# jbrea/BayesianOptimization.jl

Hardware: AMD Instinct MI355X
Metric: acquisition-candidates/sec (N=3000,d=8) (higher is better)
Workload: dtype f64

## Files before the change

bayesianoptimization.jl_amd/csrc/bohip.hip:

```cpp
#include "../../include/bohip.h"
#include "../../include/bohip_paths.h"
#include "../../include/bohip_fit.h"
#include "kernels_linalg.hip"
#include "kernels_chol.hip"
#include "kernels_exec.hip"
#include "kernels_score.hip"
#include "kernels_batch.hip"
#include "kernels_sample.hip"
#include "kernels_path.hip"
#include "kernels_ascent.hip"
#include "kernels_fit.hip"
#include "kernels_small.hip"
#include "direct_l.h"

#include <algorithm>
#include <atomic>
#include <chrono>
#include <cerrno>
#include <cmath>
#include <cstdio>
#include <cstring>
#include <limits>
#include <mutex>
#include <fcntl.h>
// ... 63 lines not shown
    int* dpieces = nullptr;
    std::vector<int> hpieces;
    int n_pieces = 0, pieces_T = -1;
    int64_t pieces_cap = 0;
    int64_t pieces_alpha = -1;
    int64_t kst_rows = 0;
    int64_t chunk_now = 0;
    int64_t score_launches = 0;
    double *dVT = nullptr, *dUT = nullptr;
    int64_t vt_rows = 0;
    double *dq = nullptr, *dmu_raw = nullptr, *dXs = nullptr, *dmu = nullptr, *dvar = nullptr, *dscore = nullptr;
    int64_t q_cap = 0, r_cap = 0, xs_cap = 0;
    Best *dblock_best = nullptr, *dbest = nullptr;
    int64_t bb_cap = 0;
    unsigned* dfz_cnt = nullptr;
    Best* dfz_best = nullptr;
    int64_t fz_cap = 0;
    bool fz_dirty = false;
    char* dpr = nullptr;
    size_t pr_bytes = 0;
    std::vector<int> hpr_pieces;
    int* pr_pieces_at = nullptr;
    unsigned* hprune_stat = nullptr;
    int prune_skip = 0;
    double* dBV = nullptr;
    int64_t bv_rows = 0, bv_ld = 0;
    char* dbatch = nullptr;
    size_t batch_bytes = 0;
    double* dgrad = nullptr;
    double asc_ftol_abs = 0.0, asc_xtol_rel = 0.0, asc_stopval = INFINITY;
    double asc_maxtime = 0.0;
    int64_t batch_hint = 0;
    double* dsplit = nullptr;
    int64_t split_cap = 0;
    const SmallFold* asc_fold = nullptr;
    bool asc_fold_done = false;
    const unsigned* asc_go = nullptr;
    double* dgparts = nullptr;
    unsigned* dgcount = nullptr;
    double* dsm = nullptr;
    size_t sm_bytes = 0;
    unsigned* dsm_cnt = nullptr;
    int sm_cnt_T = 0;
    double* hpin = nullptr;
    double* dschur = nullptr;
    AscentState asc{};
// ... 1844 lines not shown
    hipLaunchKernelGGL(k_split_combine_v, dim3((unsigned)R), dim3(256), 0, g->stream, g->dsplit, Rc * ld, ld, sp.kz, N, g->dq,
                       g->dmu_raw, want_u ? g->dVT : nullptr, ld);
    HIPCHK(hipGetLastError());
    t_end(g);
    g->q_tiles = 0;
    if (want_u) {
        t_begin(g, "split_U");
        GemmNTParams u{};
        u.A = g->dVT; u.lda = ld; u.B = g->dWT; u.ldb = ld; u.C = g->dsplit; u.ldc = ld;
        u.zA = (int64_t)sp.kz * KC; u.zB = (int64_t)sp.kz * KC; u.zC = Rc * ld;
        u.mt = (int)(Rc / TILE); u.nt64 = 2 * T; u.kc = sp.kz; u.alpha = 1.0; u.beta = 0.0;
        u.klo_from_n = 1; u.kz = sp.kz; u.ktot = T * (TILE / KC);
        CHK(launch_gemm_nt(g, u, sp.nsl));
        hipLaunchKernelGGL(k_split_combine_u, dim3((unsigned)R), dim3(256), 0, g->stream, g->dsplit, Rc * ld, ld, sp.kz, sp.nsl, N,
                           g->dUT, ld);
        HIPCHK(hipGetLastError());
        t_end(g);
    }
    return 0;
}

constexpr int PRUNE_K1 = 64;
constexpr int PRUNE_ROWS_CAP = 256;
constexpr int64_t PRUNE_R_MAX = 8192;
static int prune_tiles(int T) {
    if (g_prune_m >= 0) return g_prune_m < T ? g_prune_m : 0;
    int m = 2;
    while ((double)m * (m + 1) < 0.02 * T * (T + 1)) ++m;
    return m < T ? m : 0;
}
static std::vector<int> rows_halves(const std::vector<int>& pieces) {
    std::vector<int> out;
    if (!g_ks8) return out;
    for (int c : pieces) {
        const int rt = c & 0xffff, mode = c >> 16;
        if (mode == PIECE_UPPER_SOLO) out.push_back(rt | 1 << 17);
        else if (mode == PIECE_WHOLE) { out.push_back(rt | 1 << 16); out.push_back(rt); }
        else return {};
    }
    std::stable_sort(out.begin(), out.end(), [](int a, int b) {
        return 8 * (a & 0xffff) + ((a >> 16) & 1) * 4 > 8 * (b & 0xffff) + ((b >> 16) & 1) * 4;
    });
    return out;
}
static int rows_halves_from(const std::vector<int>& hv, int t0) {
    int n = 0;
    while (n < (int)hv.size() && (hv[n] & 0xffff) >= t0) ++n;
    return n;
}
static int launch_trigemm_rows(bohip_gp* g, const double* KsT, const int* halves, int NH, const int* list, const unsigned* cnt,
                               int cnt_max, double* q, int64_t ldq, double* mu) {
    if (NH <= 0 || cnt_max <= 0) return 0;
    RowsParams rp{};
    rp.W = g->dW; rp.ldw = g->ld; rp.KsT = KsT; rp.ldk = g->ld; rp.list = list; rp.cnt = cnt; rp.cnt_max = cnt_max;
    rp.halves = halves; rp.NH = NH; rp.G = (cnt_max + RS_COLS - 1) / RS_COLS; rp.alpha_row = g->n; rp.q = q; rp.ldq = ldq; rp.mu = mu;
    hipLaunchKernelGGL(k_trigemm_rows, dim3((unsigned)(8 * ((NH + 7) / 8) * rp.G)), dim3(RS_THREADS), RS_LDS_BYTES, g->stream, rp);
    HIPCHK(hipGetLastError());
    return 0;
}
static int launch_trigemm_on(bohip_gp* g, const double* KsT, const int* pieces, int NP, int CT, double* q, int64_t ldq, double* mu_raw,
                             FuseParams fz) {
    const int n_local = (CT + 7) / 8;
    if (NP <= 0 || CT <= 0) return 0;
    if (g->timing && g->dclk) fz.clk = g->dclk;
    if (g_ks8)
        hipLaunchKernelGGL(k_trigemm_sq<2>, dim3(8 * n_local * NP), dim3(GEMM_THREADS_8), glds3_lds_bytes<4>(), g->stream, g->dW,
                           g->ld, KsT, g->ld, pieces, NP, CT, g->n, q, ldq, mu_raw, (int64_t)0, nullptr, g->ld, fz);
    else
        hipLaunchKernelGGL(k_trigemm_sq<1>, dim3(8 * n_local * NP), dim3(GEMM_THREADS), glds3_lds_bytes<4>(), g->stream, g->dW,
                           g->ld, KsT, g->ld, pieces, NP, CT, g->n, q, ldq, mu_raw, (int64_t)0, nullptr, g->ld, fz);
    HIPCHK(hipGetLastError());
    return 0;
}
static int pruned_pass(bohip_gp* g, const double* dXs, int64_t R, int m, const AcqParams& ap, Best* d_best, int64_t best_off,
                       double* ub_host = nullptr) {
    CHK(one_time_kernel_setup());
    if (!g->hprune_stat) {
        HIPCHK(hipHostMalloc((void**)&g->hprune_stat, 64, hipHostMallocDefault));
        g->hprune_stat[0] = 0u;
    }
    const int64_t N = g->n, Npad = round_up(N + 1, TILE), Rpad = round_up(R, TILE) + TILE, ld = g->ld;
    const int T = (int)(Npad / TILE);
    const int64_t P = Npad / 64;
    CHK(ensure_pieces(g, T, N));
    std::vector<int> pa, pb;
    for (int c : g->hpieces) ((c & 0xffff) < m ? pa : pb).push_back(c);
    auto al = [](size_t b) { return (b + 255) / 256 * 256; };
    const size_t o_ks = 0, o_q2 = o_ks + al((size_t)Rpad * ld * 8), o_mu2 = o_q2 + al((size_t)2 * T * Rpad * 8),
                 o_ub = o_mu2 + al((size_t)Rpad * 8), o_l1 = o_ub + al((size_t)Rpad * 8), o_l2 = o_l1 + al((size_t)PRUNE_K1 * 4),
                 o_mark = o_l2 + al((size_t)Rpad * 4), o_cnt = o_mark + al((size_t)Rpad * 4), o_rec = o_cnt + 256,
                 o_parts = o_rec + 256, o_pc = o_parts + al((size_t)2 * P * Rpad * 8), total = o_pc + al((3 * g->hpieces.size() + 8) * 4);
    bool fresh = false;
    if (g->pr_bytes < total) {
        fresh = true;
        if (g->dpr) { HIPCHK(hipStreamSynchronize(g->stream)); HIPCHK(hipFree(g->dpr)); g->dpr = nullptr; g->pr_bytes = 0; }
        HIPCHK(hipMalloc(&g->dpr, total));
        g->pr_bytes = total;
    }
// ... 27 lines not shown
    t_end(g);
    t_begin(g, "trigemm_sq");
    FuseParams fz{};
    fz.T = T;
    CHK(launch_trigemm_on(g, g->dKsT, pcs, (int)pa.size(), (int)((R + CTILE - 1) / CTILE), g->dq, Rpad, g->dmu_raw, fz));
    PruneBound bd{};
    bd.parts = kp.parts; bd.P = P; bd.ldp = Rpad; bd.Npad = Npad; bd.q = g->dq; bd.ldq = Rpad; bd.R = R; bd.m = m;
    bd.sigma2 = sigma2; bd.beta = g->beta; bd.ap = ap; bd.ub = ub;
    hipLaunchKernelGGL(k_prune_bound, dim3((unsigned)((R + 63) / 64)), dim3(64), 0, g->stream, bd);
    if (ub_host) {
        t_end(g);
        HIPCHK(hipGetLastError());
        HIPCHK(hipMemcpyAsync(ub_host, ub, (size_t)R * 8, hipMemcpyDeviceToHost, g->stream));
        HIPCHK(hipStreamSynchronize(g->stream));
        return 0;
    }
    static_assert(PRUNE_R_MAX <= (int64_t)SELECT_THREADS * SELECT_PER, "k_prune_select holds the whole batch in one workgroup");
    hipLaunchKernelGGL(k_prune_select, dim3(1), dim3(SELECT_THREADS), 0, g->stream, (const double*)ub, R, k1, l1, mark, cnt, rec);
    HIPCHK(hipGetLastError());
    PruneFinish pf{};
    pf.q = g->dq; pf.ldq = Rpad; pf.q2 = q2; pf.ldq2 = Rpad; pf.mu2 = mu2; pf.m = m; pf.T = T; pf.sigma2 = sigma2; pf.beta = g->beta;
    pf.ap = ap; pf.rec = rec;
    const int* hvd = pcs + pa.size() + pb.size();
    for (int round = 0; round < 2; ++round) {
        const int* list = round == 0 ? l1 : l2;
        const unsigned* c = cnt + round;
        const int64_t cap = round == 0 ? k1 : R - k1;
        if (cap > 0 && nh > 0 && cap <= PRUNE_ROWS_CAP) {
            CHK(launch_trigemm_rows(g, g->dKsT, hvd, nh, list, c, (int)cap, q2, Rpad, mu2));
        } else if (cap > 0) {
            const int sq_min = nh > 0 ? PRUNE_ROWS_CAP : -1;
            hipLaunchKernelGGL(k_prune_gather, dim3((unsigned)cap), dim3(256), 0, g->stream, list, c, (const double*)g->dKsT, ld, Npad, ks2,
                               sq_min, cnt + 2);
            fz.live = cnt + 2;
            CHK(launch_trigemm_on(g, ks2, pcs + pa.size(), (int)pb.size(), (int)((cap + CTILE - 1) / CTILE), q2, Rpad, mu2, fz));
            if (nh > 0) CHK(launch_trigemm_rows(g, g->dKsT, hvd, nh, list, c, PRUNE_ROWS_CAP, q2, Rpad, mu2));
        }
        pf.list = list; pf.cnt = c;
        pf.best_out = round == 1 ? d_best : nullptr; pf.best_off = (long long)best_off;
        pf.stat = round == 1 ? g->hprune_stat : nullptr;
        pf.ub = ub; pf.mark = mark; pf.R = R; pf.list2 = round == 0 ? l2 : nullptr; pf.cnt2 = cnt + 1;
        hipLaunchKernelGGL(k_prune_finish, dim3(1), dim3(256), 0, g->stream, pf);
        HIPCHK(hipGetLastError());
    }
    t_end(g);
    return 0;
}

constexpr int PRUNE_BACKOFF = 31;
static bool prune_wanted(bohip_gp* g, int64_t R) {
    if (g->prune_skip > 0) { --g->prune_skip; return false; }
    if (g->hprune_stat) {
        const unsigned n2 = __atomic_load_n(g->hprune_stat, __ATOMIC_RELAXED);
        if ((int64_t)n2 > R / 8) {
            __atomic_store_n(g->hprune_stat, 0u, __ATOMIC_RELAXED);
            g->prune_skip = PRUNE_BACKOFF - 1;
            return false;
        }
    }
    return true;
}

static int score_core(bohip_gp* g, int acq_id, const double* acq_params, const double* dXs, int64_t R, double* d_mu,
                      double* d_var, double* d_score, Best* d_best, int64_t best_off = 0) {
    if (g->n == 0) return fail(BOHIP_E_STATE, "model has no observations");
    CHK(ensure_fresh(g));
    CHK(ensure_score_scratch(g, R));
    AcqParams ap{acq_id, 0.0, 0.0};
    if (acq_params) {
        if (acq_id != BOHIP_ACQ_MAXMEAN) ap.p0 = acq_params[0];
        if (acq_id == BOHIP_ACQ_MI) ap.p1 = acq_params[1];
    } else if (acq_id != BOHIP_ACQ_MAXMEAN) {
        return fail(BOHIP_E_ARG, "acq_params required for this acquisition");
    }
    if (path_R(g, R) <= small_limit(g) && R <= SMALL_MAX) {
        CHK(one_time_kernel_setup());
        return small_posterior(g, dXs, 0, R, false, ap, d_mu, d_var, d_score, d_best, best_off);
    }
    const SplitPlan sp = split_plan(g, R);
    if (sp.nsl > 0) {
        CHK(split_posterior(g, dXs, R, sp, false));
    } else if (int m = prune_tiles((int)(round_up(g->n + 1, TILE) / TILE));
               m > 0 && g_fuse_finish && d_best && !d_mu && !d_var && !d_score && R <= PRUNE_R_MAX && R <= g->chunk_now &&
               g->batch_hint == 0 && prune_wanted(g, R)) {
        return pruned_pass(g, dXs, R, m, ap, d_best, best_off);
    } else if (g_fuse_finish) {
        FuseParams fz{};
        fz.tile_cnt = g->dfz_cnt; fz.total_cnt = g->dfz_cnt + g->fz_cap; fz.tile_best = g->dfz_best;
        fz.tiles_total = (int)((R + CTILE - 1) / CTILE); fz.R_total = R;
        fz.sigma2 = std::exp(2.0 * g->logsig); fz.beta = g->beta; fz.ap = ap;
        fz.mu_out = d_mu; fz.var_out = d_var; fz.score_out = d_score; fz.best_out = d_best; fz.best_off = best_off;
        if (g->fz_dirty) HIPCHK(hipMemsetAsync(g->dfz_cnt, 0, (size_t)(g->fz_cap + 1 + 16) * sizeof(unsigned), g->stream));
        g->fz_dirty = true;
        const int rc = posterior_pass(g, dXs, R, fz);
        if (rc == 0) g->fz_dirty = false;
        return rc;
    } else {
        CHK(posterior_pass(g, dXs, R));
    }
    const int64_t Npad = round_up(g->n + 1, TILE), Rpad = round_up(R, TILE) + TILE;
    const int T = (int)(Npad / TILE);
    const int nb = (int)((R + 255) / 256);
    t_begin(g, "score");
    hipLaunchKernelGGL(k_score, dim3(nb), dim3(256), 0, g->stream, g->dq, Rpad, g->q_tiles, g->dmu_raw, R,
                       std::exp(2.0 * g->logsig), g->beta, ap, d_mu, d_var, d_score, d_best ? g->dblock_best : nullptr);
    if (d_best) hipLaunchKernelGGL(k_argmax_final, dim3(1), dim3(256), 0, g->stream, g->dblock_best, nb, d_best, (long long)best_off);
    HIPCHK(hipGetLastError());
    t_end(g);
// ... 1696 lines not shown
    one_time_kernel_setup();
    std::vector<int> ps;
    trigemm_pieces(T, alpha_row, ps);
    for (int i = 0; i < (int)ps.size() && i < cap; ++i) out[i] = ps[i];
    return (int)ps.size();
}
int bohip_debug_prune_bounds(bohip_gp* g, int acq_id, const double* acq_params, const double* Xs, int64_t R, double* ub) {
    if (!g || R <= 0 || !Xs || !ub || acq_id < 0 || acq_id > BOHIP_ACQ_MAXMEAN) return fail(BOHIP_E_ARG, "bad arguments");
    HIPCHK(hipSetDevice(g->device));
    if (g->n == 0) return fail(BOHIP_E_STATE, "model has no observations");
    CHK(ensure_fresh(g));
    CHK(ensure_xs(g, R));
    CHK(ensure_score_scratch(g, R));
    AcqParams ap{acq_id, 0.0, 0.0};
    if (acq_params && acq_id != BOHIP_ACQ_MAXMEAN) ap.p0 = acq_params[0];
    if (acq_params && acq_id == BOHIP_ACQ_MI) ap.p1 = acq_params[1];
    const int m = prune_tiles((int)(round_up(g->n + 1, TILE) / TILE));
    if (m == 0 || R > PRUNE_R_MAX || R > g->chunk_now || (path_R(g, R) <= small_limit(g) && R <= SMALL_MAX) || split_plan(g, R).nsl > 0)
        return fail(BOHIP_E_UNSUPPORTED, "no pruning at this size");
    HIPCHK(hipMemcpyAsync(g->dXs, Xs, (size_t)R * g->d * 8, hipMemcpyHostToDevice, g->stream));
    return pruned_pass(g, g->dXs, R, m, ap, nullptr, 0, ub);
}
int bohip_debug_trigemm_partials(bohip_gp* g, const double* Xs, int64_t R, int path, double* q_out, double* mu_out) {
    if (!g || R <= 0 || !Xs || !q_out || !mu_out || (path != 0 && path != 1)) return fail(BOHIP_E_ARG, "bad arguments");
    HIPCHK(hipSetDevice(g->device));
    if (g->n == 0) return fail(BOHIP_E_STATE, "model has no observations");
    CHK(ensure_fresh(g));
    CHK(ensure_xs(g, R));
    CHK(ensure_score_scratch(g, R));
    if (R > g->chunk_now) return fail(BOHIP_E_UNSUPPORTED, "more than one K*' chunk");
    CHK(one_time_kernel_setup());
    const int64_t N = g->n, Npad = round_up(N + 1, TILE), Rpad = round_up(R, TILE);
    const int T = (int)(Npad / TILE);
    CHK(ensure_pieces(g, T, N));
    const std::vector<int> hv = rows_halves(g->hpieces);
    if (path == 1 && hv.empty()) return fail(BOHIP_E_UNSUPPORTED, "row pieces k_trigemm_rows does not reproduce");
    HIPCHK(hipMemcpyAsync(g->dXs, Xs, (size_t)R * g->d * 8, hipMemcpyHostToDevice, g->stream));
    CHK(launch_kstar_any(g, g->dXs, 0, R, Npad, make_hyper(g)));
    std::vector<double> q((size_t)2 * T * Rpad), mu((size_t)Rpad);
    if (path == 0) {
        CHK(launch_trigemm_on(g, g->dKsT, g->dpieces, g->n_pieces, (int)((R + CTILE - 1) / CTILE), g->dq, Rpad, g->dmu_raw, FuseParams{}));
        HIPCHK(hipMemcpyAsync(q.data(), g->dq, q.size() * 8, hipMemcpyDeviceToHost, g->stream));
        HIPCHK(hipMemcpyAsync(mu.data(), g->dmu_raw, mu.size() * 8, hipMemcpyDeviceToHost, g->stream));
        HIPCHK(hipStreamSynchronize(g->stream));
        for (int t = 0; t < 2 * T; ++t) std::memcpy(q_out + (size_t)t * R, q.data() + (size_t)t * Rpad, (size_t)R * 8);
        std::memcpy(mu_out, mu.data(), (size_t)R * 8);
        return 0;
    }
    std::vector<int> list((size_t)R);
    for (int64_t i = 0; i < R; ++i) list[i] = (int)(R - 1 - i);
    const unsigned n = (unsigned)R;
    char* d = nullptr;
    const size_t o_q = 0, o_mu = o_q + q.size() * 8, o_l = o_mu + mu.size() * 8, o_h = o_l + list.size() * 4, o_c = o_h + hv.size() * 4;
    HIPCHK(hipMalloc(&d, o_c + 16));
    int rc = 0;
    hipMemcpyAsync(d + o_l, list.data(), list.size() * 4, hipMemcpyHostToDevice, g->stream);
    hipMemcpyAsync(d + o_h, hv.data(), hv.size() * 4, hipMemcpyHostToDevice, g->stream);
    hipMemcpyAsync(d + o_c, &n, 4, hipMemcpyHostToDevice, g->stream);
    rc = launch_trigemm_rows(g, g->dKsT, (const int*)(d + o_h), (int)hv.size(), (const int*)(d + o_l), (const unsigned*)(d + o_c), (int)R,
                             (double*)(d + o_q), Rpad, (double*)(d + o_mu));
    hipMemcpyAsync(q.data(), d + o_q, q.size() * 8, hipMemcpyDeviceToHost, g->stream);
    hipMemcpyAsync(mu.data(), d + o_mu, mu.size() * 8, hipMemcpyDeviceToHost, g->stream);
    const hipError_t e = hipStreamSynchronize(g->stream);
    hipFree(d);
    if (rc != 0) return rc;
    if (e != hipSuccess) return fail(BOHIP_E_HIP, hipGetErrorString(e));
    for (int t = 0; t < 2 * T; ++t)
        for (int64_t i = 0; i < R; ++i) q_out[(size_t)t * R + list[i]] = q[(size_t)t * Rpad + i];
    for (int64_t i = 0; i < R; ++i) mu_out[list[i]] = mu[i];
    return 0;
}
int64_t bohip_debug_prune_stat(bohip_gp* g) {
    if (!g || !g->hprune_stat) return -1;
    return (int64_t)__atomic_load_n(g->hprune_stat, __ATOMIC_RELAXED);
}
int bohip_debug_set_chol_inv_g(int g_new) {
    return g_chol_inv_g.exchange(std::min(64, std::max(0, g_new)));
}
int bohip_debug_exec_throughput(bohip_gp* g, unsigned qmask, int hot, int wgs, double* ms_out, double* gflop_out) {
    if (!g || !ms_out || g->n == 0) return BOHIP_E_ARG;
    hipSetDevice(g->device);
    CHK(one_time_kernel_setup());
    const int T = (int)(round_up(g->n + 1, TILE) / TILE);
    if (T <= 3) return BOHIP_E_UNSUPPORTED;
    std::vector<ExTask> all, run;
    int qb[EX_NQ + 1], qb2[EX_NQ + 1];
    exec_task_list(g->dL, g->dS, g->dW, g->dWT, g->dchol_flags, g->ld, T, g_chol_nsf, g_chol_inv_g, all, qb);
    double fl = 0.0;
    qb2[0] = 0;
    for (int qi = 0; qi < EX_NQ; ++qi) {
        if ((qmask >> qi) & 1u)
            for (int i = qb[qi]; i < qb[qi + 1]; ++i) {
                ExTask t = all[i];
                for (int d = 0; d < EX_NDEP; ++d) { t.dep_idx[d] = EX_NONE; t.dep_want[d] = 0; }
                t.sig_idx[0] = t.sig_idx[1] = EX_NONE;
                t.kc_split = 0; t.dep2_idx[0] = t.dep2_idx[1] = EX_NONE;
                if (hot && (qi == EX_QBULK || qi == EX_QWAVE)) { t.A = g->dS; t.B = g->dS + (int64_t)TILE * g->ld; }
// ... 61 lines not shown
```

bayesianoptimization.jl_amd/csrc/kernels_score.hip:

```cpp
#include "gemm_core.h"

namespace bohip {

template <bool LOW>
__device__ __forceinline__ double cov_from_r_fast(int fam, double sigma2, double r) {
    if constexpr (LOW) {
        return matern_lo_k(fam, sigma2, r);
    } else {
        if (fam == FAM_M52) {
            const double R = sqrt(r), s = sqrt(5.0) * R;
            return sigma2 * (1.0 + s + 5.0 / 3.0 * r) * exp(-s);
        }
        return sigma2 * exp(-0.5 * r);
    }
}

struct KstarParts {
    const double* alpha;
    double* parts;
    int64_t ldp;
};
__device__ __forceinline__ void swap32(double a, double b, double& x, double& y) {
    const unsigned long long ua = (unsigned long long)__double_as_longlong(a), ub = (unsigned long long)__double_as_longlong(b);
    const auto lo = __builtin_amdgcn_permlane32_swap((unsigned)ua, (unsigned)ub, false, false);
// ... 532 lines not shown
            ub = (mu_up - ap.p0 >= 0.0 ? 1.0 : acq_eval(ap, mu_up, s2)) + 0x1p-38;
            break;
        case ACQ_UCB:
        case ACQ_MI: {
            const double sb = ap.p0 >= 0.0 ? s2 : 0.0;
            const double f = acq_eval(ap, mu_up, sb);
            const double roots = ap.acq == ACQ_UCB ? sqrt(sb) : sqrt(sb + fabs(ap.p1)) + sqrt(fabs(ap.p1));
            ub = f + 0x1p-38 * (fabs(mu_up) + fabs(ap.p0) * roots + 0x1p-1000);
            break;
        }
        default:
            ub = mu_up;
    }
    pb.ub[r] = ub;
}

__device__ __forceinline__ double prune_key(double v) { return v != v ? INFINITY : v; }
__device__ __forceinline__ unsigned long long prune_key_bits(double v) {
    const double k = prune_key(v);
    const unsigned long long b = k == 0.0 ? 0ull : (unsigned long long)__double_as_longlong(k);
    return (b >> 63) ? ~b : b | 0x8000000000000000ull;
}
constexpr int SELECT_THREADS = 1024, SELECT_PER = 8;
__global__ __launch_bounds__(SELECT_THREADS) void k_prune_select(const double* __restrict__ ub, int64_t R, int k1, int* __restrict__ list1,
                                                                 int* __restrict__ mark, unsigned* __restrict__ cnt, Best* __restrict__ rec) {
    __shared__ uint4 hist[3][64];
    __shared__ unsigned long long red[2 * SELECT_THREADS / 64];
    __shared__ unsigned tot[SELECT_THREADS / 64];
    const int t = threadIdx.x, lane = t & 63, wave = t >> 6;
    const int per = (int)((R + SELECT_THREADS - 1) / SELECT_THREADS);
    unsigned long long key[SELECT_PER];
    unsigned long long kmax = 0ull, kmin = ~0ull;
#pragma unroll
    for (int i = 0; i < SELECT_PER; ++i) {
        const int64_t r = (int64_t)t * per + i;
        key[i] = (i < per && r < R) ? prune_key_bits(ub[r]) : 0ull;
        if (key[i]) { kmax = max(kmax, key[i]); kmin = min(kmin, key[i]); }
    }
    for (int o = 32; o > 0; o >>= 1) {
        kmax = max(kmax, __shfl_xor(kmax, o));
        kmin = min(kmin, __shfl_xor(kmin, o));
    }
    if (lane == 0) { red[2 * wave] = kmax; red[2 * wave + 1] = kmin; }
    if (t < 128) (&hist[0][0])[t] = make_uint4(0u, 0u, 0u, 0u);
    __syncthreads();
    for (int w = 0; w < SELECT_THREADS / 64; ++w) { kmax = max(kmax, red[2 * w]); kmin = min(kmin, red[2 * w + 1]); }
// ... 38 lines not shown
    const unsigned mine = (unsigned)ngt | (unsigned)neq << 16;
    unsigned incl = mine;
    for (int o = 1; o < 64; o <<= 1) {
        const unsigned u = __shfl_up(incl, o);
        if (lane >= o) incl += u;
    }
    if (lane == 63) tot[wave] = incl;
    __syncthreads();
    for (int w = 0; w < wave; ++w) incl += tot[w];
    int g = (int)((incl - mine) & 0xffffu), e = (int)((incl - mine) >> 16);
#pragma unroll
    for (int i = 0; i < SELECT_PER; ++i) {
        if (!key[i]) continue;
        const int64_t r = (int64_t)t * per + i;
        const bool gt = (key[i] >> hb) > thr, eq = (key[i] >> hb) == thr, in = gt || (eq && e < k);
        if (in) list1[g + min(e, k)] = (int)r;
        mark[r] = in;
        g += gt;
        e += eq;
    }
    if (t == 0) {
        cnt[0] = (unsigned)k1;
        cnt[1] = 0u;
        rec->val = -INFINITY;
        rec->idx = -1;
    }
}

__global__ __launch_bounds__(256) void k_prune_gather(const int* __restrict__ list, const unsigned* __restrict__ cnt,
                                                      const double* __restrict__ src, int64_t ld, int64_t ncols, double* __restrict__ dst,
                                                      int sq_min, unsigned* __restrict__ live_out) {
    const int i = blockIdx.x, n = (int)*cnt;
    if (i == 0 && threadIdx.x == 0) *live_out = n > sq_min ? (unsigned)n : 0u;
    if (i >= n || n <= sq_min) return;
    const d2* s = reinterpret_cast<const d2*>(src + (int64_t)list[i] * ld);
    d2* d = reinterpret_cast<d2*>(dst + (int64_t)i * ld);
    for (int64_t j = threadIdx.x; j < ncols / 2; j += 256) d[j] = s[j];
}

constexpr int RS_COLS = 8, RS_WAVES = 8, RS_THREADS = 64 * RS_WAVES, RS_DEPTH = 7;
constexpr int RS_RG = 16 / RS_WAVES;
constexpr int RS_BUF = (64 + RS_COLS) * KC;
constexpr int RS_LDS_BYTES = RS_DEPTH * RS_BUF * 8;
struct RowsParams {
    const double* W;
    int64_t ldw;
    const double* KsT;
    int64_t ldk;
    const int* list;
    const unsigned* cnt;
    int cnt_max;
    const int* halves;
    int NH, G;
    int64_t alpha_row;
    double* q;
    int64_t ldq;
    double* mu;
};
__global__ __launch_bounds__(RS_THREADS) void k_trigemm_rows(RowsParams rp) {
    __shared__ double xch[2 * 64 * RS_COLS];
    __shared__ double vb[64 * RS_COLS];
    const int xcd = blockIdx.x & 7, slot = blockIdx.x >> 3;
    const int hi = xcd + 8 * (slot / rp.G), grp = slot % rp.G;
    const int n = (int)*rp.cnt;
    if (hi >= rp.NH || n > rp.cnt_max || grp * RS_COLS >= n) return;
    const int code = __builtin_amdgcn_readfirstlane(rp.halves[hi]);
    const int rt = code & 0xffff, hh = (code >> 16) & 1;
    const bool solo = (code >> 17) & 1;
    const int tid = threadIdx.x, lane = tid & 63, wave = __builtin_amdgcn_readfirstlane(tid >> 6);
    const int h = wave / (RS_WAVES / 2), wq = wave % (RS_WAVES / 2);
    const int k = lane >> 4, b = (lane >> 2) & 3;
    const int tri_kc = 8 * rt, kc_end = tri_kc + (hh == 0 ? 4 : 8);
    const int g0 = 8 * hh + RS_RG * wq;
    extern __shared__ __attribute__((aligned(16))) double rs_ring[];
    const int prow = lane >> 3, sseg = (lane & 7) ^ prow;
    const bool has_b = wave == 0;
    const double* a_src0 = rp.W + ((int64_t)rt * TILE + 64 * hh + 8 * wave + prow) * rp.ldw + 2 * sseg;
    const int ib = grp * RS_COLS + prow;
    const double* b_src = rp.KsT + (int64_t)(ib < n ? rp.list[ib] : rp.list[0]) * rp.ldk + 2 * sseg;
    auto issue = [&](int kc, int buf) {
        kc = min(kc, kc_end - 1);
        double* d = rs_ring + buf * RS_BUF;
        __builtin_amdgcn_global_load_lds((gbl_void_ptr)(a_src0 + (int64_t)kc * KC), (lds_void_ptr)(d + 8 * wave * KC), 16, 0, 0);
        if (has_b)
            __builtin_amdgcn_global_load_lds((gbl_void_ptr)(b_src + (int64_t)kc * KC), (lds_void_ptr)(d + 64 * KC), 16, 0, 0);
    };
    auto wait_left = [&](auto left) {
        constexpr int L = decltype(left)::value;
        if (has_b) asm volatile("s_waitcnt vmcnt(%0)" ::"n"(2 * L) : "memory");
        else asm volatile("s_waitcnt vmcnt(%0)" ::"n"(L) : "memory");
    };
    const int rr = 4 * (b >> 1) + (lane & 3), cc = 4 * (b & 1) + (lane & 3), S = 4 * h + k;
    const uint32_t ring0 = (uint32_t)(uintptr_t)(__attribute__((address_space(3))) const double*)rs_ring;
    const uint32_t fa = ring0 + (uint32_t)(((8 * RS_RG * wq + rr) * KC + 2 * (S ^ rr)) * 8);
    const uint32_t fb = ring0 + (uint32_t)(((64 + cc) * KC + 2 * (S ^ cc)) * 8);
    auto frags = [&](int buf, d2 (&av)[RS_RG], d2 (&bv)[1]) {
        const uint32_t off = (uint32_t)(buf * RS_BUF * 8);
        av[0] = ds_read128<0>(fa + off);
        av[1] = ds_read128<1024>(fa + off);
        bv[0] = ds_read128<0>(fb + off);
    };
    auto landed = [&](d2 (&av)[RS_RG], d2 (&bv)[1]) {
        asm volatile("s_waitcnt lgkmcnt(0)" : "+v"(av[0]), "+v"(av[1]), "+v"(bv[0]));
    };
    double acc[RS_RG][1], acc2[RS_RG][1];
    auto run = [&](auto solo_tag) {
        constexpr bool SOLO = decltype(solo_tag)::value;
#pragma unroll
        for (int i = 0; i < RS_RG; ++i)
#pragma unroll
            for (int j = 0; j < 1; ++j) acc[i][j] = acc2[i][j] = 0.0;
        auto step = [&](int kc, int cur, const d2 (&av)[RS_RG], const d2 (&bv)[1], d2 (&avn)[RS_RG], d2 (&bvn)[1]) {
            wait_left(std::integral_constant<int, RS_DEPTH - 2>{});
            __builtin_amdgcn_s_barrier();
            __builtin_amdgcn_sched_barrier(0);
            issue(kc + RS_DEPTH, cur);
            frags(cur + 1 == RS_DEPTH ? 0 : cur + 1, avn, bvn);
            __builtin_amdgcn_sched_barrier(0);
            const int skip = kc >= tri_kc ? 2 * (kc - tri_kc) + h - g0 : 0;
#pragma unroll
            for (int i = 0; i < RS_RG; ++i) {
                if (skip > i) continue;
                if constexpr (SOLO) {
                    mma_row<1, 1>(av[i], bv, acc[i]);
                    mma_row<1, 2>(av[i], bv, acc2[i]);
                } else {
                    mma_row<1, 0>(av[i], bv, acc[i]);
                }
            }
            landed(avn, bvn);
            __builtin_amdgcn_sched_barrier(0);
        };
#pragma unroll
        for (int p = 0; p < RS_DEPTH; ++p) issue(p, p);
        d2 av0[RS_RG], bv0[1], av1[RS_RG], bv1[1];
        wait_left(std::integral_constant<int, RS_DEPTH - 1>{});
        __builtin_amdgcn_s_barrier();
        __builtin_amdgcn_sched_barrier(0);
        frags(0, av0, bv0);
        landed(av0, bv0);
        __builtin_amdgcn_sched_barrier(0);
        int cur = 0;
        for (int kc = 0; kc < kc_end; kc += 2) {
            step(kc, cur, av0, bv0, av1, bv1);
            cur = cur + 1 == RS_DEPTH ? 0 : cur + 1;
            step(kc + 1, cur, av1, bv1, av0, bv0);
            cur = cur + 1 == RS_DEPTH ? 0 : cur + 1;
        }
        asm volatile("s_waitcnt vmcnt(0)" ::: "memory");
    };
    if (solo) run(std::true_type{});
    else run(std::false_type{});
    if (h == 1) {
#pragma unroll
        for (int i = 0; i < RS_RG; ++i)
#pragma unroll
            for (int j = 0; j < 1; ++j) {
                xch[((wq * RS_RG + i)  + j) * 64 + lane] = acc[i][j];
                xch[64 * RS_COLS + ((wq * RS_RG + i)  + j) * 64 + lane] = acc2[i][j];
            }
    }
    __syncthreads();
    if (h == 0) {
#pragma unroll
        for (int i = 0; i < RS_RG; ++i)
#pragma unroll
            for (int j = 0; j < 1; ++j) {
                const double a1 = xch[((wq * RS_RG + i)  + j) * 64 + lane];
                double v = acc[i][j] + a1;
                if (solo) {
                    const double o1 = xch[64 * RS_COLS + ((wq * RS_RG + i)  + j) * 64 + lane];
                    v = v + (acc2[i][j] + o1);
                }
                const int row = 8 * (RS_RG * wq + i) + 4 * (b >> 1) + k, col = 8 * j + 4 * (b & 1) + (lane & 3);
                vb[row * RS_COLS + col] = v;
            }
    }
    __syncthreads();
    if (wave >= 1) return;
    const int col = 8 * wave + 4 * (b & 1) + (lane & 3), i_list = grp * RS_COLS + col;
    const int64_t row_base = (int64_t)rt * TILE + 64 * hh;
    double s = 0.0;
#pragma unroll
    for (int mi = 0; mi < 8; ++mi) {
        const int row = 8 * mi + 4 * (b >> 1) + k;
        const double v = vb[row * RS_COLS + col];
        if (row_base + row == rp.alpha_row) {
            if (i_list < n) rp.mu[i_list] = v;
        } else {
            s = sq_step(s, v);
        }
    }
    s = sq_tree(s);
    if (lane < 8 && i_list < n) {
        rp.q[(int64_t)(2 * rt + hh) * rp.ldq + i_list] = s;
        if (solo) rp.q[(int64_t)(2 * rt + 1) * rp.ldq + i_list] = 0.0;
    }
}

struct PruneFinish {
    const int* list;
    const unsigned* cnt;
    const double *q, *q2, *mu2;
    int64_t ldq, ldq2;
    int m, T;
    double sigma2, beta;
    AcqParams ap;
    Best* rec;
    Best* best_out;
    long long best_off;
    unsigned* stat;
    const double* ub;
    const int* mark;
    int64_t R;
    int* list2;
    unsigned* cnt2;
};
__global__ __launch_bounds__(256) void k_prune_finish(PruneFinish pf) {
#pragma clang fp contract(off)
    __shared__ Best sh[4];
    __shared__ double tail_L;
    __shared__ unsigned tail_n;
    const int n = (int)*pf.cnt;
    double v = -INFINITY;
    long long idx = -1;
    for (int i = threadIdx.x; i < n; i += 256) {
        const int64_t r = pf.list[i];
        double q = 0.0;
        for (int t0 = 0; t0 < pf.T; t0 += 8) {
            double a[8], b[8];
#pragma unroll
            for (int u = 0; u < 8; ++u) {
                const int t = min(t0 + u, pf.T - 1);
                const double* src = t < pf.m ? pf.q + r : pf.q2 + i;
                const int64_t ld = t < pf.m ? pf.ldq : pf.ldq2;
                a[u] = src[(int64_t)(2 * t) * ld];
                b[u] = src[(int64_t)(2 * t + 1) * ld];
            }
#pragma unroll
            for (int u = 0; u < 8; ++u)
                if (t0 + u < pf.T) q += a[u] + b[u];
        }
        double s2 = pf.sigma2 - q;
        if (s2 < 0.0) s2 = 0.0;
        const double mu = pf.beta + pf.mu2[i];
        const double f = acq_eval(pf.ap, mu, s2);
        if (better(f, r, v, idx)) { v = f; idx = r; }
    }
    block_argmax(v, idx, sh);
    if (threadIdx.x == 0) {
        const Best b = *pf.rec;
        if (better(b.val, b.idx, v, idx)) { v = b.val; idx = b.idx; }
        pf.rec->val = idx >= 0 ? v : -INFINITY;
        pf.rec->idx = idx;
        if (pf.best_out) {
            pf.best_out->val = idx >= 0 ? v : -INFINITY;
            pf.best_out->idx = idx >= 0 ? idx + pf.best_off : -1;
        }
        if (pf.stat) *pf.stat = (unsigned)n;
        tail_L = idx >= 0 ? v : -INFINITY;
        tail_n = 0u;
    }
    if (!pf.list2) return;
    __syncthreads();
    const double L = tail_L;
    for (int64_t r0 = threadIdx.x; r0 < pf.R; r0 += 8 * 256) {
        int mk[8];
        double u[8];
#pragma unroll
        for (int i = 0; i < 8; ++i) {
            const int64_t r = min(r0 + 256 * i, pf.R - 1);
            mk[i] = pf.mark[r];
            u[i] = pf.ub[r];
        }
#pragma unroll
        for (int i = 0; i < 8; ++i)
            if (r0 + 256 * i < pf.R && !mk[i] && !(u[i] < L)) pf.list2[atomicAdd(&tail_n, 1u)] = (int)(r0 + 256 * i);
    }
    __syncthreads();
    if (threadIdx.x == 0) *pf.cnt2 = tail_n;
}

__global__ __launch_bounds__(256) void k_reduce_records(const Best* __restrict__ all, int nrec, int S, Best* __restrict__ out) {
    const int s = blockIdx.x * 256 + threadIdx.x;
    if (s >= S) return;
    double v = -INFINITY;
    long long idx = -1;
    for (int r = 0; r < nrec; ++r) {
        const Best b = all[(int64_t)r * S + s];
        if (better(b.val, b.idx, v, idx)) { v = b.val; idx = b.idx; }
    }
    out[s].val = idx >= 0 ? v : -INFINITY;
    out[s].idx = idx;
}

__device__ __forceinline__ void acq_partials(const AcqParams& a, double mu, double s2, double& dmu, double& ds2) {
    const double inv_sqrt_2pi = 0.3989422804014327;
    switch (a.acq) {
        case ACQ_EI: {
            if (s2 == 0.0) { dmu = mu > a.p0 ? 1.0 : 0.0; ds2 = 0.0; return; }
            const double D = mu - a.p0, s = sqrt(s2), z = D / s;
            const double Phi = 0.5 * (1.0 + erf(z / sqrt(2.0))), phi = inv_sqrt_2pi * exp(-0.5 * z * z);
            dmu = Phi + D * phi / s - z * phi / s;
// ... 260 lines not shown
```

Baseline: 24.69 million.

## Fuse prune finish into row trigemm via last-block arrival and loop groups

The pruned pass now runs the finish reduction inside k_trigemm_rows: the last workgroup to arrive, counted by an atomic arrival counter, executes the finish body. This removes separate k_prune_finish launches. Round two uses a fixed number of groups that loop over a device-side count of any size, replacing the host-sized gather and square-trigemm path unless a long form is chosen from earlier prune statistics. The row kernel's LDS ring deepens to 8 and is advanced in pairs with one barrier per two chunks. This adds atomic and fence synchronisation and puts more serial work on a few workgroups.

Result: faster. 26.73 million (median of 6 runs) (+8.3%).

```diff
diff --git a/bayesianoptimization.jl_amd/csrc/bohip.hip b/bayesianoptimization.jl_amd/csrc/bohip.hip
--- a/bayesianoptimization.jl_amd/csrc/bohip.hip
+++ b/bayesianoptimization.jl_amd/csrc/bohip.hip
@@ -109,6 +109,9 @@
     std::vector<int> hpr_pieces;
     int* pr_pieces_at = nullptr;
     unsigned* hprune_stat = nullptr;
+    unsigned prune_seen = 0;
+    bool prune_retry = false;
+    int prune_r2_form = -1;
     int prune_skip = 0;
     double* dBV = nullptr;
     int64_t bv_rows = 0, bv_ld = 0;
@@ -1999,6 +2002,7 @@
 
 constexpr int PRUNE_K1 = 64;
 constexpr int PRUNE_ROWS_CAP = 256;
+constexpr int PRUNE_R2_GROUPS = 8;
 constexpr int64_t PRUNE_R_MAX = 8192;
 static int prune_tiles(int T) {
     if (g_prune_m >= 0) return g_prune_m < T ? g_prune_m : 0;
@@ -2026,11 +2030,14 @@
     return n;
 }
 static int launch_trigemm_rows(bohip_gp* g, const double* KsT, const int* halves, int NH, const int* list, const unsigned* cnt,
-                               int cnt_max, double* q, int64_t ldq, double* mu) {
+                               int cnt_max, double* q, int64_t ldq, double* mu, int groups = 0, const PruneFinish* pf = nullptr,
+                               unsigned* arrive = nullptr) {
     if (NH <= 0 || cnt_max <= 0) return 0;
     RowsParams rp{};
     rp.W = g->dW; rp.ldw = g->ld; rp.KsT = KsT; rp.ldk = g->ld; rp.list = list; rp.cnt = cnt; rp.cnt_max = cnt_max;
-    rp.halves = halves; rp.NH = NH; rp.G = (cnt_max + RS_COLS - 1) / RS_COLS; rp.alpha_row = g->n; rp.q = q; rp.ldq = ldq; rp.mu = mu;
+    rp.halves = halves; rp.NH = NH; rp.G = groups > 0 ? groups : (cnt_max + RS_COLS - 1) / RS_COLS;
+    rp.alpha_row = g->n; rp.q = q; rp.ldq = ldq; rp.mu = mu;
+    if (pf) { rp.finish = 1; rp.arrive = arrive; rp.pf = *pf; }
     hipLaunchKernelGGL(k_trigemm_rows, dim3((unsigned)(8 * ((NH + 7) / 8) * rp.G)), dim3(RS_THREADS), RS_LDS_BYTES, g->stream, rp);
     HIPCHK(hipGetLastError());
     return 0;
@@ -2050,7 +2057,7 @@
     return 0;
 }
 static int pruned_pass(bohip_gp* g, const double* dXs, int64_t R, int m, const AcqParams& ap, Best* d_best, int64_t best_off,
-                       double* ub_host = nullptr) {
+                       double* ub_host = nullptr, bool long_form = false) {
     CHK(one_time_kernel_setup());
     if (!g->hprune_stat) {
         HIPCHK(hipHostMalloc((void**)&g->hprune_stat, 64, hipHostMallocDefault));
@@ -2124,24 +2131,42 @@
     pf.q = g->dq; pf.ldq = Rpad; pf.q2 = q2; pf.ldq2 = Rpad; pf.mu2 = mu2; pf.m = m; pf.T = T; pf.sigma2 = sigma2; pf.beta = g->beta;
     pf.ap = ap; pf.rec = rec;
     const int* hvd = pcs + pa.size() + pb.size();
+    pf.ub = ub; pf.mark = mark; pf.R = R; pf.cnt2 = cnt + 1; pf.best_off = (long long)best_off;
+    if (nh > 0) {
+        pf.list = l1; pf.cnt = cnt; pf.list2 = l2; pf.best_out = d_best; pf.stat = g->hprune_stat;
+        CHK(launch_trigemm_rows(g, g->dKsT, hvd, nh, l1, cnt, k1, q2, Rpad, mu2, 0, &pf, cnt + PRUNE_ARRIVE));
+        const int64_t cap = R - k1;
+        pf.list = l2; pf.cnt = cnt + 1; pf.list2 = nullptr;
+        if (cap > 0 && !long_form) {
+            CHK(launch_trigemm_rows(g, g->dKsT, hvd, nh, l2, cnt + 1, INT_MAX, q2, Rpad, mu2, PRUNE_R2_GROUPS, &pf, cnt + PRUNE_ARRIVE + 1));
+        } else if (cap > 0) {
+            if (cap > PRUNE_ROWS_CAP) {
+                hipLaunchKernelGGL(k_prune_gather, dim3((unsigned)cap), dim3(256), 0, g->stream, (const int*)l2, (const unsigned*)(cnt + 1),
+                                   (const double*)g->dKsT, ld, Npad, ks2, PRUNE_ROWS_CAP, cnt + 2);
+                fz.live = cnt + 2;
+                CHK(launch_trigemm_on(g, ks2, pcs + pa.size(), (int)pb.size(), (int)((cap + CTILE - 1) / CTILE), q2, Rpad, mu2, fz));
+            }
+            CHK(launch_trigemm_rows(g, g->dKsT, hvd, nh, l2, cnt + 1, (int)std::min<int64_t>(cap, PRUNE_ROWS_CAP), q2, Rpad, mu2));
+            hipLaunchKernelGGL(k_prune_finish, dim3(1), dim3(256), 0, g->stream, pf);
+            HIPCHK(hipGetLastError());
+        }
+        t_end(g);
+        return 0;
+    }
     for (int round = 0; round < 2; ++round) {
         const int* list = round == 0 ? l1 : l2;
         const unsigned* c = cnt + round;
         const int64_t cap = round == 0 ? k1 : R - k1;
-        if (cap > 0 && nh > 0 && cap <= PRUNE_ROWS_CAP) {
-            CHK(launch_trigemm_rows(g, g->dKsT, hvd, nh, list, c, (int)cap, q2, Rpad, mu2));
-        } else if (cap > 0) {
-            const int sq_min = nh > 0 ? PRUNE_ROWS_CAP : -1;
+        if (cap > 0) {
             hipLaunchKernelGGL(k_prune_gather, dim3((unsigned)cap), dim3(256), 0, g->stream, list, c, (const double*)g->dKsT, ld, Npad, ks2,
-                               sq_min, cnt + 2);
+                               -1, cnt + 2);
             fz.live = cnt + 2;
             CHK(launch_trigemm_on(g, ks2, pcs + pa.size(), (int)pb.size(), (int)((cap + CTILE - 1) / CTILE), q2, Rpad, mu2, fz));
-            if (nh > 0) CHK(launch_trigemm_rows(g, g->dKsT, hvd, nh, list, c, PRUNE_ROWS_CAP, q2, Rpad, mu2));
         }
         pf.list = list; pf.cnt = c;
-        pf.best_out = round == 1 ? d_best : nullptr; pf.best_off = (long long)best_off;
+        pf.best_out = round == 1 ? d_best : nullptr;
         pf.stat = round == 1 ? g->hprune_stat : nullptr;
-        pf.ub = ub; pf.mark = mark; pf.R = R; pf.list2 = round == 0 ? l2 : nullptr; pf.cnt2 = cnt + 1;
+        pf.list2 = round == 0 ? l2 : nullptr;
         hipLaunchKernelGGL(k_prune_finish, dim3(1), dim3(256), 0, g->stream, pf);
         HIPCHK(hipGetLastError());
     }
@@ -2152,11 +2177,14 @@
 constexpr int PRUNE_BACKOFF = 31;
 static bool prune_wanted(bohip_gp* g, int64_t R) {
     if (g->prune_skip > 0) { --g->prune_skip; return false; }
+    g->prune_seen = 0u;
     if (g->hprune_stat) {
         const unsigned n2 = __atomic_load_n(g->hprune_stat, __ATOMIC_RELAXED);
+        g->prune_seen = n2;
         if ((int64_t)n2 > R / 8) {
             __atomic_store_n(g->hprune_stat, 0u, __ATOMIC_RELAXED);
             g->prune_skip = PRUNE_BACKOFF - 1;
+            g->prune_retry = true;
             return false;
         }
     }
@@ -2185,7 +2213,9 @@
     } else if (int m = prune_tiles((int)(round_up(g->n + 1, TILE) / TILE));
                m > 0 && g_fuse_finish && d_best && !d_mu && !d_var && !d_score && R <= PRUNE_R_MAX && R <= g->chunk_now &&
                g->batch_hint == 0 && prune_wanted(g, R)) {
-        return pruned_pass(g, dXs, R, m, ap, d_best, best_off);
+        const bool want_long = g->prune_retry || g->prune_seen > (unsigned)PRUNE_ROWS_CAP;
+        g->prune_retry = false;
+        return pruned_pass(g, dXs, R, m, ap, d_best, best_off, nullptr, g->prune_r2_form < 0 ? want_long : g->prune_r2_form == 1);
     } else if (g_fuse_finish) {
         FuseParams fz{};
         fz.tile_cnt = g->dfz_cnt; fz.total_cnt = g->dfz_cnt + g->fz_cap; fz.tile_best = g->dfz_best;
@@ -3928,7 +3958,7 @@
     return pruned_pass(g, g->dXs, R, m, ap, nullptr, 0, ub);
 }
 int bohip_debug_trigemm_partials(bohip_gp* g, const double* Xs, int64_t R, int path, double* q_out, double* mu_out) {
-    if (!g || R <= 0 || !Xs || !q_out || !mu_out || (path != 0 && path != 1)) return fail(BOHIP_E_ARG, "bad arguments");
+    if (!g || R <= 0 || !Xs || !q_out || !mu_out || path < 0 || path > 2) return fail(BOHIP_E_ARG, "bad arguments");
     HIPCHK(hipSetDevice(g->device));
     if (g->n == 0) return fail(BOHIP_E_STATE, "model has no observations");
     CHK(ensure_fresh(g));
@@ -3940,7 +3970,7 @@
     const int T = (int)(Npad / TILE);
     CHK(ensure_pieces(g, T, N));
     const std::vector<int> hv = rows_halves(g->hpieces);
-    if (path == 1 && hv.empty()) return fail(BOHIP_E_UNSUPPORTED, "row pieces k_trigemm_rows does not reproduce");
+    if (path != 0 && hv.empty()) return fail(BOHIP_E_UNSUPPORTED, "row pieces k_trigemm_rows does not reproduce");
     HIPCHK(hipMemcpyAsync(g->dXs, Xs, (size_t)R * g->d * 8, hipMemcpyHostToDevice, g->stream));
     CHK(launch_kstar_any(g, g->dXs, 0, R, Npad, make_hyper(g)));
     std::vector<double> q((size_t)2 * T * Rpad), mu((size_t)Rpad);
@@ -3964,7 +3994,7 @@
     hipMemcpyAsync(d + o_h, hv.data(), hv.size() * 4, hipMemcpyHostToDevice, g->stream);
     hipMemcpyAsync(d + o_c, &n, 4, hipMemcpyHostToDevice, g->stream);
     rc = launch_trigemm_rows(g, g->dKsT, (const int*)(d + o_h), (int)hv.size(), (const int*)(d + o_l), (const unsigned*)(d + o_c), (int)R,
-                             (double*)(d + o_q), Rpad, (double*)(d + o_mu));
+                             (double*)(d + o_q), Rpad, (double*)(d + o_mu), path == 2 ? 1 : 0);
     hipMemcpyAsync(q.data(), d + o_q, q.size() * 8, hipMemcpyDeviceToHost, g->stream);
     hipMemcpyAsync(mu.data(), d + o_mu, mu.size() * 8, hipMemcpyDeviceToHost, g->stream);
     const hipError_t e = hipStreamSynchronize(g->stream);
@@ -3979,6 +4009,11 @@
 int64_t bohip_debug_prune_stat(bohip_gp* g) {
     if (!g || !g->hprune_stat) return -1;
     return (int64_t)__atomic_load_n(g->hprune_stat, __ATOMIC_RELAXED);
+}
+int bohip_debug_prune_round2_form(bohip_gp* g, int form) {
+    if (!g || form < -1 || form > 1) return fail(BOHIP_E_ARG, "bad arguments");
+    g->prune_r2_form = form;
+    return 0;
 }
 int bohip_debug_set_chol_inv_g(int g_new) {
     return g_chol_inv_g.exchange(std::min(64, std::max(0, g_new)));
diff --git a/bayesianoptimization.jl_amd/csrc/kernels_score.hip b/bayesianoptimization.jl_amd/csrc/kernels_score.hip
--- a/bayesianoptimization.jl_amd/csrc/kernels_score.hip
+++ b/bayesianoptimization.jl_amd/csrc/kernels_score.hip
@@ -578,6 +578,7 @@
     return (b >> 63) ? ~b : b | 0x8000000000000000ull;
 }
 constexpr int SELECT_THREADS = 1024, SELECT_PER = 8;
+constexpr int PRUNE_ARRIVE = 4;
 __global__ __launch_bounds__(SELECT_THREADS) void k_prune_select(const double* __restrict__ ub, int64_t R, int k1, int* __restrict__ list1,
                                                                  int* __restrict__ mark, unsigned* __restrict__ cnt, Best* __restrict__ rec) {
     __shared__ uint4 hist[3][64];
@@ -662,6 +663,8 @@
     if (t == 0) {
         cnt[0] = (unsigned)k1;
         cnt[1] = 0u;
+        cnt[PRUNE_ARRIVE] = 0u;
+        cnt[PRUNE_ARRIVE + 1] = 0u;
         rec->val = -INFINITY;
         rec->idx = -1;
     }
@@ -678,7 +681,105 @@
     for (int64_t j = threadIdx.x; j < ncols / 2; j += 256) d[j] = s[j];
 }
 
-constexpr int RS_COLS = 8, RS_WAVES = 8, RS_THREADS = 64 * RS_WAVES, RS_DEPTH = 7;
+struct PruneFinish {
+    const int* list;
+    const unsigned* cnt;
+    const double *q, *q2, *mu2;
+    int64_t ldq, ldq2;
+    int m, T;
+    double sigma2, beta;
+    AcqParams ap;
+    Best* rec;
+    Best* best_out;
+    long long best_off;
+    unsigned* stat;
+    const double* ub;
+    const int* mark;
+    int64_t R;
+    int* list2;
+    unsigned* cnt2;
+};
+template <int NT>
+__device__ __forceinline__ void prune_finish_body(const PruneFinish& pf, Best* sh, double* tail_L, unsigned* tail_n) {
+#pragma clang fp contract(off)
+    const int n = (int)*pf.cnt;
+    double v = -INFINITY;
+    long long idx = -1;
+    for (int i = threadIdx.x; i < n; i += NT) {
+        const int64_t r = pf.list[i];
+        double q = 0.0;
+        for (int t0 = 0; t0 < pf.T; t0 += 8) {
+            double a[8], b[8];
+#pragma unroll
+            for (int u = 0; u < 8; ++u) {
+                const int t = min(t0 + u, pf.T - 1);
+                const double* src = t < pf.m ? pf.q + r : pf.q2 + i;
+                const int64_t ld = t < pf.m ? pf.ldq : pf.ldq2;
+                a[u] = src[(int64_t)(2 * t) * ld];
+                b[u] = src[(int64_t)(2 * t + 1) * ld];
+            }
+#pragma unroll
+            for (int u = 0; u < 8; ++u)
+                if (t0 + u < pf.T) q += a[u] + b[u];
+        }
+        double s2 = pf.sigma2 - q;
+        if (s2 < 0.0) s2 = 0.0;
+        const double mu = pf.beta + pf.mu2[i];
+        const double f = acq_eval(pf.ap, mu, s2);
+        if (better(f, r, v, idx)) { v = f; idx = r; }
+    }
+    block_argmax(v, idx, sh);
+    const bool last_round = !pf.list2;
+    if (threadIdx.x == 0) {
+        const Best b = *pf.rec;
+        if (better(b.val, b.idx, v, idx)) { v = b.val; idx = b.idx; }
+        pf.rec->val = idx >= 0 ? v : -INFINITY;
+        pf.rec->idx = idx;
+        if (pf.best_out && last_round) {
+            pf.best_out->val = idx >= 0 ? v : -INFINITY;
+            pf.best_out->idx = idx >= 0 ? idx + pf.best_off : -1;
+        }
+        if (pf.stat && last_round) *pf.stat = (unsigned)n;
+        *tail_L = idx >= 0 ? v : -INFINITY;
+        *tail_n = 0u;
+    }
+    if (last_round) return;
+    __syncthreads();
+    const double L = *tail_L;
+    for (int64_t r0 = threadIdx.x; r0 < pf.R; r0 += 8 * NT) {
+        int mk[8];
+        double u[8];
+#pragma unroll
+        for (int i = 0; i < 8; ++i) {
+            const int64_t r = min(r0 + NT * i, pf.R - 1);
+            mk[i] = pf.mark[r];
+            u[i] = pf.ub[r];
+        }
+#pragma unroll
+        for (int i = 0; i < 8; ++i)
+            if (r0 + NT * i < pf.R && !mk[i] && !(u[i] < L)) pf.list2[atomicAdd(tail_n, 1u)] = (int)(r0 + NT * i);
+    }
+    __syncthreads();
+    if (threadIdx.x == 0) {
+        const unsigned n2 = *tail_n;
+        *pf.cnt2 = n2;
+        if (n2 == 0u) {
+            if (pf.best_out) {
+                pf.best_out->val = idx >= 0 ? v : -INFINITY;
+                pf.best_out->idx = idx >= 0 ? idx + pf.best_off : -1;
+            }
+            if (pf.stat) *pf.stat = 0u;
+        }
+    }
+}
+__global__ __launch_bounds__(256) void k_prune_finish(PruneFinish pf) {
+    __shared__ Best sh[4];
+    __shared__ double tail_L;
+    __shared__ unsigned tail_n;
+    prune_finish_body<256>(pf, sh, &tail_L, &tail_n);
+}
+
+constexpr int RS_COLS = 8, RS_WAVES = 8, RS_THREADS = 64 * RS_WAVES, RS_DEPTH = 8;
 constexpr int RS_RG = 16 / RS_WAVES;
 constexpr int RS_BUF = (64 + RS_COLS) * KC;
 constexpr int RS_LDS_BYTES = RS_DEPTH * RS_BUF * 8;
@@ -696,14 +797,17 @@
     double* q;
     int64_t ldq;
     double* mu;
+    int finish;
+    unsigned* arrive;
+    PruneFinish pf;
 };
 __global__ __launch_bounds__(RS_THREADS) void k_trigemm_rows(RowsParams rp) {
     __shared__ double xch[2 * 64 * RS_COLS];
     __shared__ double vb[64 * RS_COLS];
     const int xcd = blockIdx.x & 7, slot = blockIdx.x >> 3;
-    const int hi = xcd + 8 * (slot / rp.G), grp = slot % rp.G;
+    const int hi = xcd + 8 * (slot / rp.G), grp0 = slot % rp.G;
     const int n = (int)*rp.cnt;
-    if (hi >= rp.NH || n > rp.cnt_max || grp * RS_COLS >= n) return;
+    if (hi >= rp.NH || n > rp.cnt_max || grp0 * RS_COLS >= n) return;
     const int code = __builtin_amdgcn_readfirstlane(rp.halves[hi]);
     const int rt = code & 0xffff, hh = (code >> 16) & 1;
     const bool solo = (code >> 17) & 1;
@@ -716,8 +820,7 @@
     const int prow = lane >> 3, sseg = (lane & 7) ^ prow;
     const bool has_b = wave == 0;
     const double* a_src0 = rp.W + ((int64_t)rt * TILE + 64 * hh + 8 * wave + prow) * rp.ldw + 2 * sseg;
-    const int ib = grp * RS_COLS + prow;
-    const double* b_src = rp.KsT + (int64_t)(ib < n ? rp.list[ib] : rp.list[0]) * rp.ldk + 2 * sseg;
+    const double* b_src = nullptr;
     auto issue = [&](int kc, int buf) {
         kc = min(kc, kc_end - 1);
         double* d = rs_ring + buf * RS_BUF;
@@ -750,13 +853,7 @@
         for (int i = 0; i < RS_RG; ++i)
 #pragma unroll
             for (int j = 0; j < 1; ++j) acc[i][j] = acc2[i][j] = 0.0;
-        auto step = [&](int kc, int cur, const d2 (&av)[RS_RG], const d2 (&bv)[1], d2 (&avn)[RS_RG], d2 (&bvn)[1]) {
-            wait_left(std::integral_constant<int, RS_DEPTH - 2>{});
-            __builtin_amdgcn_s_barrier();
-            __builtin_amdgcn_sched_barrier(0);
-            issue(kc + RS_DEPTH, cur);
-            frags(cur + 1 == RS_DEPTH ? 0 : cur + 1, avn, bvn);
-            __builtin_amdgcn_sched_barrier(0);
+        auto mmas = [&](int kc, const d2 (&av)[RS_RG], const d2 (&bv)[1]) {
             const int skip = kc >= tri_kc ? 2 * (kc - tri_kc) + h - g0 : 0;
 #pragma unroll
             for (int i = 0; i < RS_RG; ++i) {
@@ -768,13 +865,12 @@
                     mma_row<1, 0>(av[i], bv, acc[i]);
                 }
             }
-            landed(avn, bvn);
-            __builtin_amdgcn_sched_barrier(0);
         };
-#pragma unroll
-        for (int p = 0; p < RS_DEPTH; ++p) issue(p, p);
+        static_assert(RS_DEPTH % 2 == 0, "a pair of chunks per barrier: the ring turns in pairs");
+#pragma unroll
+        for (int p = 0; p < RS_DEPTH - 1; ++p) issue(p, p);
         d2 av0[RS_RG], bv0[1], av1[RS_RG], bv1[1];
-        wait_left(std::integral_constant<int, RS_DEPTH - 1>{});
+        wait_left(std::integral_constant<int, RS_DEPTH - 2>{});
         __builtin_amdgcn_s_barrier();
         __builtin_amdgcn_sched_barrier(0);
         frags(0, av0, bv0);
@@ -782,13 +878,29 @@
         __builtin_amdgcn_sched_barrier(0);
         int cur = 0;
         for (int kc = 0; kc < kc_end; kc += 2) {
-            step(kc, cur, av0, bv0, av1, bv1);
-            cur = cur + 1 == RS_DEPTH ? 0 : cur + 1;
-            step(kc + 1, cur, av1, bv1, av0, bv0);
-            cur = cur + 1 == RS_DEPTH ? 0 : cur + 1;
+            wait_left(std::integral_constant<int, RS_DEPTH - 4>{});
+            __builtin_amdgcn_s_barrier();
+            __builtin_amdgcn_sched_barrier(0);
+            const int prev = cur == 0 ? RS_DEPTH - 1 : cur - 1, b1 = cur + 1, b2 = cur + 2 == RS_DEPTH ? 0 : cur + 2;
+            issue(kc + RS_DEPTH - 1, prev);
+            issue(kc + RS_DEPTH, cur);
+            frags(b1, av1, bv1);
+            __builtin_amdgcn_sched_barrier(0);
+            mmas(kc, av0, bv0);
+            landed(av1, bv1);
+            __builtin_amdgcn_sched_barrier(0);
+            frags(b2, av0, bv0);
+            __builtin_amdgcn_sched_barrier(0);
+            mmas(kc + 1, av1, bv1);
+            landed(av0, bv0);
+            __builtin_amdgcn_sched_barrier(0);
+            cur = b2;
         }
         asm volatile("s_waitcnt vmcnt(0)" ::: "memory");
     };
+    for (int grp = grp0; grp * RS_COLS < n; grp += rp.G) {
+    const int ib = grp * RS_COLS + prow;
+    b_src = rp.KsT + (int64_t)(ib < n ? rp.list[ib] : rp.list[0]) * rp.ldk + 2 * sseg;
     if (solo) run(std::true_type{});
     else run(std::false_type{});
     if (h == 1) {
@@ -817,7 +929,7 @@
             }
     }
     __syncthreads();
-    if (wave >= 1) return;
+    if (wave == 0) {
     const int col = 8 * wave + 4 * (b & 1) + (lane & 3), i_list = grp * RS_COLS + col;
     const int64_t row_base = (int64_t)rt * TILE + 64 * hh;
     double s = 0.0;
@@ -836,89 +948,28 @@
         rp.q[(int64_t)(2 * rt + hh) * rp.ldq + i_list] = s;
         if (solo) rp.q[(int64_t)(2 * rt + 1) * rp.ldq + i_list] = 0.0;
     }
-}
-
-struct PruneFinish {
-    const int* list;
-    const unsigned* cnt;
-    const double *q, *q2, *mu2;
-    int64_t ldq, ldq2;
-    int m, T;
-    double sigma2, beta;
-    AcqParams ap;
-    Best* rec;
-    Best* best_out;
-    long long best_off;
-    unsigned* stat;
-    const double* ub;
-    const int* mark;
-    int64_t R;
-    int* list2;
-    unsigned* cnt2;
-};
-__global__ __launch_bounds__(256) void k_prune_finish(PruneFinish pf) {
-#pragma clang fp contract(off)
-    __shared__ Best sh[4];
-    __shared__ double tail_L;
-    __shared__ unsigned tail_n;
-    const int n = (int)*pf.cnt;
-    double v = -INFINITY;
-    long long idx = -1;
-    for (int i = threadIdx.x; i < n; i += 256) {
-        const int64_t r = pf.list[i];
-        double q = 0.0;
-        for (int t0 = 0; t0 < pf.T; t0 += 8) {
-            double a[8], b[8];
-#pragma unroll
-            for (int u = 0; u < 8; ++u) {
-                const int t = min(t0 + u, pf.T - 1);
-                const double* src = t < pf.m ? pf.q + r : pf.q2 + i;
-                const int64_t ld = t < pf.m ? pf.ldq : pf.ldq2;
-                a[u] = src[(int64_t)(2 * t) * ld];
-                b[u] = src[(int64_t)(2 * t + 1) * ld];
-            }
-#pragma unroll
-            for (int u = 0; u < 8; ++u)
-                if (t0 + u < pf.T) q += a[u] + b[u];
-        }
-        double s2 = pf.sigma2 - q;
-        if (s2 < 0.0) s2 = 0.0;
-        const double mu = pf.beta + pf.mu2[i];
-        const double f = acq_eval(pf.ap, mu, s2);
-        if (better(f, r, v, idx)) { v = f; idx = r; }
-    }
-    block_argmax(v, idx, sh);
-    if (threadIdx.x == 0) {
-        const Best b = *pf.rec;
-        if (better(b.val, b.idx, v, idx)) { v = b.val; idx = b.idx; }
-        pf.rec->val = idx >= 0 ? v : -INFINITY;
-        pf.rec->idx = idx;
-        if (pf.best_out) {
-            pf.best_out->val = idx >= 0 ? v : -INFINITY;
-            pf.best_out->idx = idx >= 0 ? idx + pf.best_off : -1;
-        }
-        if (pf.stat) *pf.stat = (unsigned)n;
-        tail_L = idx >= 0 ? v : -INFINITY;
-        tail_n = 0u;
-    }
-    if (!pf.list2) return;
-    __syncthreads();
-    const double L = tail_L;
-    for (int64_t r0 = threadIdx.x; r0 < pf.R; r0 += 8 * 256) {
-        int mk[8];
-        double u[8];
-#pragma unroll
-        for (int i = 0; i < 8; ++i) {
-            const int64_t r = min(r0 + 256 * i, pf.R - 1);
-            mk[i] = pf.mark[r];
-            u[i] = pf.ub[r];
-        }
-#pragma unroll
-        for (int i = 0; i < 8; ++i)
-            if (r0 + 256 * i < pf.R && !mk[i] && !(u[i] < L)) pf.list2[atomicAdd(&tail_n, 1u)] = (int)(r0 + 256 * i);
-    }
-    __syncthreads();
-    if (threadIdx.x == 0) *pf.cnt2 = tail_n;
+    asm volatile("s_waitcnt vmcnt(0)" ::: "memory");
+    }
+    __syncthreads();
+    }
+    if (!rp.finish) return;
+    unsigned* flag = reinterpret_cast<unsigned*>(xch + 64);
+    if (tid == 0) {
+        __builtin_amdgcn_fence(__ATOMIC_RELEASE, "agent");
+        asm volatile("s_waitcnt vmcnt(0)" ::: "memory");
+        const unsigned want = (unsigned)rp.NH * (unsigned)min(rp.G, (n + RS_COLS - 1) / RS_COLS);
+        const bool last = __hip_atomic_fetch_add(rp.arrive, 1u, __ATOMIC_RELAXED, __HIP_MEMORY_SCOPE_AGENT) == want - 1u;
+        if (last) __hip_atomic_store(rp.arrive, 0u, __ATOMIC_RELAXED, __HIP_MEMORY_SCOPE_AGENT);
+        *flag = last;
+    }
+    __syncthreads();
+    if (!*flag) return;
+    if (tid == 0) {
+        __builtin_amdgcn_fence(__ATOMIC_ACQUIRE, "agent");
+        asm volatile("s_waitcnt vmcnt(0)" ::: "memory");
+    }
+    __syncthreads();
+    prune_finish_body<RS_THREADS>(rp.pf, reinterpret_cast<Best*>(xch), xch + 32, reinterpret_cast<unsigned*>(xch + 40));
 }
 
 __global__ __launch_bounds__(256) void k_reduce_records(const Best* __restrict__ all, int nrec, int S, Best* __restrict__ out) {
```
